# pinellolab/GRAFIMO

Hardware: AMD Instinct MI355X
Metric: scored haplotype k-mers/sec (higher is better)
Workload: dtype int32

## Files before the change

grafimo_amd/_native.py:

```python
import ctypes
import os

import numpy as np

_HERE = os.path.dirname(os.path.abspath(__file__))
LIB_PATH = os.environ.get("GRAFIMO_HIP_LIB") or os.path.join(_HERE, "csrc", "libgrafimo_hip.so")

GFM_OK = 0
GFM_ERR_INVALID = -1
GFM_ERR_ASSERT = -2
GFM_ERR_HIP = -3
GFM_ERR_NOMEM = -4
GFM_ERR_NODEVICE = -5
GFM_ERR_IO = -6
GFM_ERR_OVERFLOW = -7
GFM_NO_SELECT = 2**31 - 1
GFM_FLAG_RESET_HITS = 1
GFM_FLAG_CLEAR_HIST = 2
GFM_FLAG_CALLER_ORDERS_REUSE = 4
GFM_MAX_WIDTH = 64
GFM_BEST_ROW_BITS = 44
GFM_GRAPH_FORWARD_ONLY = 1
GFM_TSV_NO_NODEPATH = 1
GFM_WORKSPACE_RING = 4
# ... 15 lines not shown
P = ctypes.POINTER

PROTOTYPES = {
    "gfm_abi_version": (c_int, []),
    "gfm_last_error": (ctypes.c_char_p, []),
    "gfm_device_count": (c_int, [P(c_int)]),
    "gfm_set_device": (c_int, [c_int]),
    "gfm_compute_log_odds": (c_int, [c_void_p, c_int, c_void_p, c_void_p]),
    "gfm_scale_pwm": (c_int, [c_void_p, c_int, c_void_p, P(c_int), P(c_int), P(c_int), P(c_double)]),
    "gfm_comp_pval_mat": (c_int, [c_void_p, c_int, c_void_p, c_void_p]),
    "gfm_comp_pval_mat_many": (c_int, [c_int, c_void_p, c_void_p, c_void_p, c_void_p]),
    "gfm_motif_create": (c_int, [c_void_p, c_int, c_void_p, c_int, c_int, c_double, c_void_p, P(c_void_p)]),
    "gfm_motif_create_many": (c_int, [c_int, c_void_p, c_void_p, c_void_p, c_void_p, c_void_p, c_void_p, c_void_p,
                                      c_void_p]),
    "gfm_motif_destroy": (None, [c_void_p]),
    "gfm_motif_width": (c_int, [c_void_p]),
    "gfm_motif_table_len": (c_int, [c_void_p]),
    "gfm_motif_score_range": (c_int, [c_void_p, P(c_i32), P(c_i32)]),
    "gfm_motif_tables": (c_int, [c_void_p, c_void_p, c_void_p]),
    "gfm_motif_pvalue_cutoff": (c_int, [c_void_p, c_double, P(c_i32)]),
    "gfm_motif_annotate": (c_int, [c_void_p, c_void_p, c_i64, c_void_p, c_void_p]),
    "gfm_score_kmers": (c_int, [c_void_p, c_void_p, c_i64, c_void_p, c_void_p, c_i32, c_i64,
                                c_void_p, c_i64, c_void_p, ctypes.c_uint32, c_void_p, c_void_p]),
    "gfm_score_kmers_multi": (c_int, [c_void_p, c_int, c_void_p, c_i64, c_void_p, c_void_p, c_void_p, c_i64,
                                      c_void_p, c_void_p, c_void_p, ctypes.c_uint32, c_void_p]),
    "gfm_score_kmers_multi_plan": (c_int, [c_void_p, c_int, c_void_p, c_void_p, c_void_p]),
    "gfm_profile_enable": (c_int, [c_void_p, c_int, c_int]),
    "gfm_profile_read": (c_int, [c_void_p, c_void_p, c_int, P(c_int)]),
    "gfm_profile_mark_tail": (c_int, [c_void_p, c_void_p]),
    "gfm_profile_read_tail": (c_int, [c_void_p, c_void_p, c_int, P(c_int)]),
    "gfm_calibrate_stream": (c_int, [c_int, c_i64, c_int, c_int, P(c_double), P(c_double)]),
    "gfm_qvalue_table": (c_int, [c_void_p, c_void_p, c_double, c_int, c_void_p, c_void_p, c_void_p,
                                 ctypes.c_uint32, c_void_p]),
    "gfm_qvalue_table_multi": (c_int, [c_void_p, c_int, c_void_p, c_double, c_int, c_void_p, c_void_p, c_void_p,
                                       ctypes.c_uint32, c_void_p]),
    "gfm_select_hits": (c_int, [c_void_p, c_void_p, c_i64, c_void_p, c_i64, c_void_p, c_i64, c_void_p,
                                ctypes.c_uint32, c_void_p]),
    "gfm_select_hits_from": (c_int, [c_void_p, c_void_p, c_i64, c_void_p, c_i64, c_void_p, c_i64, c_void_p,
                                     c_void_p, c_i64, c_void_p, c_void_p]),
    "gfm_region_ids": (c_int, [c_void_p, c_i32, c_i64, c_void_p, c_void_p]),
    "gfm_region_best": (c_int, [c_void_p, c_i64, c_void_p, c_i32, c_void_p, c_i32, c_void_p, c_i64, c_void_p, c_void_p]),
    "gfm_locus_max_workspace": (c_i64, [c_i64]),
    "gfm_locus_max": (c_int, [c_void_p, c_i64, c_void_p, c_i32, c_void_p, c_void_p, c_void_p, c_i32, c_void_p, c_void_p,
                              c_i64, c_void_p, c_void_p]),
    "gfm_scan_host": (c_int, [c_void_p, c_void_p, c_i64, c_double, c_int, c_int, c_i64, c_void_p,
                              c_void_p, c_void_p, c_void_p, c_void_p, P(c_i64)]),
# ... 175 lines not shown
```

grafimo_amd/csrc/grafimo_hip.hip:

```cpp

#include <hip/hip_runtime.h>

#include <algorithm>
#include <atomic>
#include <cmath>
#include <cstdarg>
#include <cstdint>
#include <cstdio>
#include <cstdlib>
#include <cstring>
#include <new>
#include <string>
#include <vector>

#include "grafimo_hip.h"

#define GFM_API extern "C" __attribute__((visibility("default")))

#include "gfm_hit_sort.hpp"
#include "gfm_common.hpp"
#include "gfm_score_kernels.hpp"
#include "gfm_quad_launch.hpp"
#include "gfm_stats_kernels.hpp"

struct gfm_motif {
    int W = 0, L = 0, min_val = 0, scale = 1, ndw = 0;
    double offset = 0.0;
    int lo = 0, hi = 0, nb = 0;
    int hlo = 0, hnb = 0;
    int q_waves = kWavesPerWG;
    int part_nb = 0;
    struct Window { int bins, lo; double mass; };
    std::vector<Window> windows;
    int device = 0;
    int n_cu = 256;
    int max_slabs = 0;
    int sel_slabs = 0;
    int reserve_cus = kReserveCUs;
    size_t lds_bytes = 0;
    std::vector<int64_t> sm;
    double bg[4] = {0, 0, 0, 0};
    std::vector<double> h_ptable;
    unsigned char *d_slab = nullptr;
    uint16_t *d_tab = nullptr;
    unsigned *d_ftab = nullptr;
    double *d_pmf = nullptr;
    double *d_ptable = nullptr;
    unsigned *d_partials[kWorkspaces] = {};
    unsigned *d_spill[kWorkspaces] = {};
    long long *d_resid[kWorkspaces] = {};
    int *d_resid_n[kWorkspaces] = {};
    QWork *d_qwork = nullptr;
    double *d_qscratch = nullptr;
    hipStream_t q_stream[kQStreams] = {};
    int q_streams_used = 0;
    unsigned long long q_last_use[kQStreams] = {}, q_calls = 0;
    hipEvent_t ev_selected = nullptr;
    hipStream_t sel_last_stream = nullptr;
    bool sel_valid = false;
    HitCtl *d_ctl = nullptr;
    unsigned call_no = 0;
    hipStream_t last_st = nullptr, last_tail = nullptr;
    unsigned same_pair_run = 0;
    hipEvent_t ev_scored[kWorkspaces] = {};
    hipEvent_t ev_posted[kWorkspaces] = {};
    bool posted_valid[kWorkspaces] = {};
    long long *d_sel_resid = nullptr;
    int *d_sel_resid_n = nullptr;
    HitCtl *d_sel_ctl = nullptr;
    unsigned sel_call_no = 0;
    std::vector<hipEvent_t> ev0, ev1;
    int ev_next = 0, ev_used = 0, ev_every = 1;
    unsigned ev_calls = 0;
    std::vector<hipEvent_t> tev0, tev1;
    int ev_last = -1;
    int tail_pending = -1;
    std::vector<int> tail_order;
};

namespace {

int ensure_device()
{
// ... 470 lines not shown
            for (int c = 0; c < 4; ++c) {
                const unsigned fwd = (unsigned)sm[(size_t)row_of_code[c] * W + j];
                const unsigned rc_ = (unsigned)sm[(size_t)row_of_code[c ^ 2] * W + (W - 1 - j)];
                ftab[(size_t)j * 8 + c] = fwd | (rc_ << 16);
            }
    }
    const size_t o_ftab = carve(ftab.size() * sizeof(unsigned));
    const size_t o_pmf = carve(sizeof(double) * (size_t)m->L);
    const size_t o_ptable = carve(sizeof(double) * (size_t)m->L);
    const size_t o_dp = carve(sizeof(double) * 2 * (size_t)m->L);
    const size_t o_qwork = carve(sizeof(QWork) * kQStreams);
    const size_t o_qscratch = carve(sizeof(double) * (size_t)m->L * kQStreams);
    size_t o_partials[kWorkspaces], o_resid[kWorkspaces], o_resid_n[kWorkspaces], o_spill[kWorkspaces];
    for (int i = 0; i < kWorkspaces; ++i) {
        o_partials[i] = carve(sizeof(unsigned) * (size_t)m->max_slabs * (size_t)(m->part_nb + 1));
        o_resid[i] = carve(sizeof(long long) * (size_t)m->max_slabs * kResidPerWG);
        o_resid_n[i] = carve(sizeof(int) * (size_t)m->max_slabs);
    }
    const size_t o_sel_resid = carve(sizeof(long long) * (size_t)m->sel_slabs * kResidPerWG);
    const size_t o_sel_resid_n = carve(sizeof(int) * (size_t)m->sel_slabs);
    const size_t o_zero = slab_bytes;
    for (int i = 0; i < kWorkspaces; ++i) o_spill[i] = carve(sizeof(unsigned) * (size_t)m->nb * (size_t)kSpillCopies);
    const size_t o_ctl = carve(sizeof(HitCtl));
    const size_t o_sel_ctl = carve(sizeof(HitCtl));
    HIP_TRY(hipMalloc(&m->d_slab, slab_bytes));
    HIP_TRY(hipMemsetAsync(m->d_slab + o_zero, 0, slab_bytes - o_zero, nullptr));
    m->d_tab = reinterpret_cast<uint16_t *>(m->d_slab + o_tab);
    m->d_ftab = reinterpret_cast<unsigned *>(m->d_slab + o_ftab);
    m->d_pmf = reinterpret_cast<double *>(m->d_slab + o_pmf);
    m->d_ptable = reinterpret_cast<double *>(m->d_slab + o_ptable);
    m->d_qwork = reinterpret_cast<QWork *>(m->d_slab + o_qwork);
    m->d_qscratch = reinterpret_cast<double *>(m->d_slab + o_qscratch);
    for (int i = 0; i < kWorkspaces; ++i) {
        m->d_partials[i] = reinterpret_cast<unsigned *>(m->d_slab + o_partials[i]);
        m->d_resid[i] = reinterpret_cast<long long *>(m->d_slab + o_resid[i]);
        m->d_resid_n[i] = reinterpret_cast<int *>(m->d_slab + o_resid_n[i]);
        m->d_spill[i] = reinterpret_cast<unsigned *>(m->d_slab + o_spill[i]);
        HIP_TRY(hipEventCreateWithFlags(&m->ev_scored[i], hipEventDisableTiming | hipEventReleaseToDevice));
        HIP_TRY(hipEventCreateWithFlags(&m->ev_posted[i], hipEventDisableTiming | hipEventReleaseToDevice));
    }
    HIP_TRY(hipEventCreateWithFlags(&m->ev_selected, hipEventDisableTiming));
    m->d_sel_resid = reinterpret_cast<long long *>(m->d_slab + o_sel_resid);
    m->d_sel_resid_n = reinterpret_cast<int *>(m->d_slab + o_sel_resid_n);
    m->d_ctl = reinterpret_cast<HitCtl *>(m->d_slab + o_ctl);
    m->d_sel_ctl = reinterpret_cast<HitCtl *>(m->d_slab + o_sel_ctl);
    *d_rows = reinterpret_cast<double *>(m->d_slab + o_dp);

    HIP_TRY(hipMemcpyAsync(m->d_tab, tab.data(), tab.size() * sizeof(uint16_t), hipMemcpyHostToDevice, nullptr));
    HIP_TRY(hipMemcpyAsync(m->d_ftab, ftab.data(), ftab.size() * sizeof(unsigned), hipMemcpyHostToDevice, nullptr));
    return GFM_OK;
}

int motif_finish(gfm_motif *m)
{
    const int W = m->W;
    long long room16, room8;
    score_rooms(W, &room16, &room8);
    constexpr double kWindowMass16 = 0.9999;
    m->q_waves = kWavesPerWG;
    if (m->nb <= room16) {
        m->hnb = m->nb;
    } else if (room16 >= 256 && best_window(m, (int)room16).mass >= kWindowMass16) {
        m->hnb = (int)room16;
    } else {
        m->q_waves = kWavesPerWG / 2;
        m->hnb = (int)std::min<long long>(m->nb, room8);
    }
// ... 190 lines not shown
    if (!m || !cutoff) return fail(GFM_ERR_INVALID, "NULL argument");
    int a = 0, b = m->L;
    while (a < b) {
        const int mid = (a + b) / 2;
        if (m->h_ptable[mid] < threshold) b = mid; else a = mid + 1;
    }
    *cutoff = a;
    return GFM_OK;
}

GFM_API int gfm_motif_annotate(gfm_motif_t m, const int32_t *scores, int64_t n, double *lo_out,
                               double *p_out)
{
    if (!m || (!scores && n)) return fail(GFM_ERR_INVALID, "NULL argument");
    for (int64_t i = 0; i < n; ++i) {
        const int s = scores[i];
        if (s < 0 || s >= m->L) return fail(GFM_ERR_INVALID, "score %d outside the table", s);
        if (lo_out) lo_out[i] = ((double)s / (double)m->scale) + ((double)m->W * m->offset);
        if (p_out) p_out[i] = m->h_ptable[s];
    }
    return GFM_OK;
}

GFM_API int gfm_score_kmers(gfm_motif_t m, const uint8_t *d_kmers, int64_t n, int32_t *d_scores,
                            uint64_t *d_hist, int32_t select_cutoff, int64_t row_base,
                            int64_t *d_hit_rows, int64_t hit_capacity, uint64_t *d_hit_count,
                            uint32_t flags, void *stream, void *tail_stream)
{
    if (!m) return fail(GFM_ERR_INVALID, "motif is NULL");
    if (n < 0) return fail(GFM_ERR_INVALID, "negative row count");
    hipStream_t st = static_cast<hipStream_t>(stream);
    hipStream_t tail = tail_stream ? static_cast<hipStream_t>(tail_stream) : st;
    const bool split = tail != st;
    if (n == 0) {
        if ((flags & GFM_FLAG_RESET_HITS) && d_hit_count) {
            if (split) {
                HIP_TRY(hipEventRecord(m->ev_scored[0], st));
                HIP_TRY(hipStreamWaitEvent(tail, m->ev_scored[0], 0));
            }
            HIP_TRY(hipMemsetAsync(d_hit_count, 0, sizeof(uint64_t), tail));
        }
        return GFM_OK;
    }
    if (!d_kmers) return fail(GFM_ERR_INVALID, "NULL device buffer");
    {
        int dev = -1;
        HIP_TRY(hipGetDevice(&dev));
        if (dev != m->device)
            return fail(GFM_ERR_INVALID, "the motif lives on device %d, the current device is %d", m->device, dev);
    }
    if ((reinterpret_cast<uintptr_t>(d_kmers) & 15u) != 0)
        return fail(GFM_ERR_INVALID, "d_kmers must be 16-byte aligned");
    if ((reinterpret_cast<uintptr_t>(d_scores) & 3u) != 0)
        return fail(GFM_ERR_INVALID, "d_scores must be 4-byte aligned");
    if (!d_scores && !d_hist && select_cutoff == GFM_NO_SELECT)
        return fail(GFM_ERR_INVALID, "nothing to do: no scores, no histogram, no selection");
    if (n > (int64_t)kQuadRows * 0x7fffff00ll)
        return fail(GFM_ERR_INVALID, "too many rows for one launch (split the batch)");
    const bool select = select_cutoff != GFM_NO_SELECT;
    if (select && (!d_hit_rows || !d_hit_count))
        return fail(GFM_ERR_INVALID, "selection requested without hit buffers");
    const int use_hist = d_hist ? 1 : 0;
    const long long nchunks = (n + kQuadRows - 1) / kQuadRows;
    const long long want = (nchunks + m->q_waves - 1) / m->q_waves;
// ... 22 lines not shown
    const bool caller_orders = (flags & GFM_FLAG_CALLER_ORDERS_REUSE) && same_owner && m->same_pair_run >= (unsigned)kWorkspaces;
    m->same_pair_run = same_owner ? m->same_pair_run + 1 : 1;
    m->last_st = st;
    m->last_tail = tail;
    if (m->posted_valid[ws] && !caller_orders)
        HIP_TRY(hipStreamWaitEvent(st, m->ev_posted[ws], 0));
    if (split && select && !reset && m->posted_valid[ws_prev])
        HIP_TRY(hipStreamWaitEvent(st, m->ev_posted[ws_prev], 0));
    ScoreArgs<1> args{};
    args.store_through = d_scores ? score_store_through(n, 1) : 2;
    fill_motif_args(args.m[0], m, ws, slot, use_hist, m->hlo, m->hnb, select_cutoff, d_scores,
                    reinterpret_cast<long long *>(d_hit_rows), hit_capacity,
                    reset ? nullptr : reinterpret_cast<unsigned long long *>(d_hit_count));
    hipEvent_t scored = split ? m->ev_scored[ws] : nullptr;
    int rc = dispatch_quad(m->W, 1, m, d_kmers, n, row_base, &args, m->lds_bytes, nslabs, m->q_waves, st, false,
                           split ? &scored : nullptr);
    if (rc) return rc;
    if (split) HIP_TRY(hipStreamWaitEvent(tail, scored, 0));
    m->tail_pending = -1;
    if (split && m->ev_last >= 0 && !m->tev0.empty()) {
        HIP_TRY(hipEventRecord(m->tev0[m->ev_last], tail));
        m->tail_pending = m->ev_last;
    }
    rc = launch_post(m, m->d_partials[ws], nslabs, reinterpret_cast<unsigned long long *>(d_hist),
                     m->hlo, m->hnb, m->d_spill[ws], m->d_resid[ws], m->d_resid_n[ws], select ? nslabs : 0, m->d_ctl, slot,
                     reinterpret_cast<long long *>(d_hit_rows), hit_capacity,
                     reinterpret_cast<unsigned long long *>(d_hit_count), tail);
    if (rc) return rc;
    if (split) {
        HIP_TRY(hipEventRecord(m->ev_posted[ws], tail));
        m->posted_valid[ws] = true;
    } else {
        m->posted_valid[ws] = false;
    }
    return GFM_OK;
}

GFM_API int gfm_score_kmers_multi(const gfm_motif_t *motifs, int n_motifs, const uint8_t *d_kmers,
                                  int64_t n, int32_t *const *d_scores, uint64_t *const *d_hist,
                                  const int32_t *select_cutoffs, int64_t row_base,
                                  int64_t *const *d_hit_rows, const int64_t *hit_capacity,
                                  uint64_t *const *d_hit_count, uint32_t flags, void *stream)
{
    if (!motifs || n_motifs < 1) return fail(GFM_ERR_INVALID, "NULL argument");
    if (n < 0) return fail(GFM_ERR_INVALID, "negative row count");
    hipStream_t st = static_cast<hipStream_t>(stream);
    const bool reset = (flags & GFM_FLAG_RESET_HITS) != 0;
    bool no_scores = d_scores == nullptr;
    if (d_scores) {
        int n_null = 0;
        for (int i = 0; i < n_motifs; ++i) n_null += d_scores[i] ? 0 : 1;
        if (n_null != 0 && n_null != n_motifs) return fail(GFM_ERR_INVALID, "d_scores: every entry or none (scores are stored for all motifs of a call or for none)");
        no_scores = n_null == n_motifs;
    }
    for (int i = 0; i < n_motifs; ++i) {
        if (!motifs[i]) return fail(GFM_ERR_INVALID, "motif %d is NULL", i);
        if (motifs[i]->W != motifs[0]->W)
            return fail(GFM_ERR_INVALID, "motifs of one batched launch must share their width (%d vs %d)",
// ... 161 lines not shown
        HIP_TRY(hipEventElapsedTime(&h_ms[i], m->tev0[slot], m->tev1[slot]));
    }
    *n_out = used;
    m->tail_order.clear();
    return GFM_OK;
}

GFM_API int gfm_profile_read(gfm_motif_t m, float *h_ms, int capacity, int *n_out)
{
    if (!m || !n_out || (!h_ms && capacity)) return fail(GFM_ERR_INVALID, "NULL argument");
    const int slots = (int)m->ev0.size();
    const int used = std::min(m->ev_used, capacity);
    for (int i = 0; i < used; ++i) {
        const int slot = ((m->ev_next - m->ev_used + i) % slots + slots) % slots;
        HIP_TRY(hipEventSynchronize(m->ev1[slot]));
        HIP_TRY(hipEventElapsedTime(&h_ms[i], m->ev0[slot], m->ev1[slot]));
    }
    *n_out = used;
    m->ev_used = 0;
    return GFM_OK;
}

namespace {
int launch_qtables(const gfm_motif_t *motifs, int count, uint64_t *const *d_hist, double threshold, int on_qvalue,
                   double *const *d_qtable, int32_t *const *d_cutoff, uint64_t *const *d_nrows, uint32_t flags,
                   hipStream_t st)
{
    QJobs jobs{};
    jobs.threshold = threshold;
    jobs.on_qvalue = on_qvalue;
    int max_blk = 0;
    for (int k = 0; k < count; ++k) {
        gfm_motif *m = motifs[k];
        QJob &q = jobs.j[k];
        q.hist = reinterpret_cast<const unsigned long long *>(d_hist[k]);
        q.ptable = m->d_ptable;
        int qs = 0;
        while (qs < m->q_streams_used && m->q_stream[qs] != st) ++qs;
        if (qs == m->q_streams_used) {
            if (qs < kQStreams) {
                ++m->q_streams_used;
            } else {
                qs = 0;
                for (int c = 1; c < kQStreams; ++c)
                    if (m->q_last_use[c] < m->q_last_use[qs]) qs = c;
            }
            m->q_stream[qs] = st;
        }
        m->q_last_use[qs] = ++m->q_calls;
        q.ws = m->d_qwork + qs;
        q.qtable = (d_qtable && d_qtable[k]) ? d_qtable[k] : m->d_qscratch + (size_t)qs * (size_t)m->L;
        q.cutoff = d_cutoff ? d_cutoff[k] : nullptr;
        q.nrows = d_nrows ? reinterpret_cast<unsigned long long *>(d_nrows[k]) : nullptr;
        q.clear = (flags & GFM_FLAG_CLEAR_HIST) ? reinterpret_cast<unsigned long long *>(d_hist[k]) : nullptr;
        q.L = m->L; q.lo = m->lo; q.hi = m->hi; q.min_val = m->min_val;
        q.nblk = (m->nb + kQThreads - 1) / kQThreads;
        max_blk = std::max(max_blk, q.nblk);
    }
    const dim3 grid((unsigned)max_blk, (unsigned)count);
    hipLaunchKernelGGL(q_count_kernel, grid, dim3(kQThreads), 0, st, jobs);
    hipLaunchKernelGGL(q_raw_kernel, grid, dim3(kQThreads), 0, st, jobs);
    hipLaunchKernelGGL(q_final_kernel, grid, dim3(kQThreads), 0, st, jobs);
    HIP_TRY(hipGetLastError());
    return GFM_OK;
}
}

GFM_API int gfm_qvalue_table(gfm_motif_t m, uint64_t *d_hist, double threshold, int on_qvalue,
                             double *d_qtable, int32_t *d_cutoff, uint64_t *d_nrows, uint32_t flags,
                             void *stream)
{
    if (!m || !d_hist) return fail(GFM_ERR_INVALID, "NULL argument");
// ... 239 lines not shown
```

grafimo_amd/device.py:

```python
import ctypes
from collections import OrderedDict
from typing import List, Optional

import numpy as np

from . import _native as nv

RANGE = nv.RANGE


def _torch():
    import torch
    return torch


_FP_WEIGHTS = {}


def _fingerprint(pmf) -> tuple:
    words = np.ascontiguousarray(pmf, dtype=np.float64).view(np.uint64)
    n = len(words)
    if not n:
        return (0, 0, 0)
    w = _FP_WEIGHTS.get(n)
# ... 200 lines not shown
    def fused_views(self, device):
        v = getattr(self, "_fused_views", None)
        w = self.fused_workspace(device)
        if v is None or v[3] is not w:
            torch, L = _torch(), self.L
            v = self._fused_views = (w[:L], w[L:2 * L].view(torch.float64), w[2 * L:2 * L + 1].view(torch.int32)[:1], w)
        return v[:3]

    def score(self, kmers, scores, hist=None, select_cutoff=None, row_base=0, hit_rows=None,
              hit_count=None, stream=None, reset_hits=False, tail_stream=None):
        n = int(kmers.shape[0])
        assert kmers.is_contiguous() and kmers.dtype == _torch().uint8
        assert n == 0 or kmers.shape[1] == self.width
        cut = nv.GFM_NO_SELECT if select_cutoff is None else int(select_cutoff)
        nv.check(nv.lib().gfm_score_kmers(
            self._h, kmers.data_ptr() if n else None, n, scores.data_ptr() if (n and scores is not None) else None,
            hist.data_ptr() if hist is not None else None, cut, int(row_base),
            hit_rows.data_ptr() if hit_rows is not None else None,
            int(hit_rows.numel()) if hit_rows is not None else 0,
            hit_count.data_ptr() if hit_count is not None else None,
            nv.GFM_FLAG_RESET_HITS if reset_hits else 0, _stream_ptr(stream),
            _stream_ptr(tail_stream) if tail_stream is not None else None))

    def qvalue_table(self, hist, threshold, on_qvalue, qtable=None, cutoff=None, nrows=None,
                     stream=None, clear_hist=False):
        nv.check(nv.lib().gfm_qvalue_table(
            self._h, hist.data_ptr(), float(threshold), int(bool(on_qvalue)),
            qtable.data_ptr() if qtable is not None else None,
            cutoff.data_ptr() if cutoff is not None else None,
            nrows.data_ptr() if nrows is not None else None,
            nv.GFM_FLAG_CLEAR_HIST if clear_hist else 0, _stream_ptr(stream)))

    def select_hits(self, scores, cutoff, hit_rows, hit_count, row_base=0, stream=None,
                    reset_hits=False):
        n = int(scores.numel())
        nv.check(nv.lib().gfm_select_hits(self._h, scores.data_ptr() if n else None, n, cutoff.data_ptr(),
                                          int(row_base), hit_rows.data_ptr(), int(hit_rows.numel()),
                                          hit_count.data_ptr(),
                                          nv.GFM_FLAG_RESET_HITS if reset_hits else 0,
                                          _stream_ptr(stream)))

    def select_hits_from(self, scores, cutoff, cand_rows, cand_count, hit_rows, hit_count, row_base=0, stream=None):
        n = int(scores.numel())
        nv.check(nv.lib().gfm_select_hits_from(self._h, scores.data_ptr() if n else None, n, cutoff.data_ptr(),
                                               int(row_base), cand_rows.data_ptr(), int(cand_rows.numel()),
                                               cand_count.data_ptr(), hit_rows.data_ptr(), int(hit_rows.numel()),
# ... 145 lines not shown
```

grafimo_amd/scan.py:

```python
from typing import Optional

import numpy as np

from . import _native as _nv
from .device import DeviceMotif, _torch

HIT_SCORE_BITS = 20


class ScanSlot:

    def __init__(self, dm: DeviceMotif, n_rows: int, hit_capacity: int, device, scores=None):
        torch = _torch()
        self.n_rows = int(n_rows)
        self.hit_capacity = int(hit_capacity)
        self.scores = scores if scores is not None else torch.empty(self.n_rows, dtype=torch.int32, device=device)
        self.hist = torch.zeros(dm.L, dtype=torch.int64, device=device)
        self.qtable = torch.empty(dm.L, dtype=torch.float64, device=device)
        self.cutoff = torch.zeros(1, dtype=torch.int32, device=device)
        self.nrows = torch.zeros(1, dtype=torch.int64, device=device)
        self.hits = torch.zeros(self.hit_capacity + 1, dtype=torch.int64, device=device)
        self.best = None
        self.cand = None
        self.p_cand_count = self.p_cand_rows = None
# ... 96 lines not shown
        torch = _torch()
        lib = self._lib
        dm = self.dm
        slot = self.slots[self._turn % len(self.slots)]
        self._turn += 1
        main = torch.cuda.current_stream(self.device)
        main_p = main.cuda_stream
        tail = self.side if self.side is not None else main
        tail_p = self._side_p if self.side is not None else main_p
        if slot.used:
            if self.host_paced:
                slot.done.synchronize()
            else:
                main.wait_event(slot.done)
        slot.used = True
        if self._score_ring < len(self.slots) and (on_qvalue or self._regions is not None):
            prev = self.slots[(self._turn - 1 - self._score_ring) % len(self.slots)]
            if prev.used and self._turn > self._score_ring:
                prev.done.synchronize()
        n = int(d_kmers.shape[0])
        kp = d_kmers.data_ptr() if n else None
        h = dm.handle
        use_cand = on_qvalue and self.candidates
        if not on_qvalue:
            key = float(threshold)
            cut = self._cutoffs.get(key)
            if cut is None:
                cut = self._cutoffs[key] = dm.pvalue_cutoff(key)
            _nv.check(lib.gfm_score_kmers(h, kp, n, slot.p_scores, slot.p_hist if want_qvalues else None,
                                          cut, int(row_base), slot.p_hit_rows, slot.hit_capacity,
                                          slot.p_hit_count, _nv.GFM_FLAG_RESET_HITS | self._reuse_flag, main_p, tail_p))
        elif not use_cand:
            _nv.check(lib.gfm_score_kmers(h, kp, n, slot.p_scores, slot.p_hist, _nv.GFM_NO_SELECT, 0,
                                          None, 0, None, self._reuse_flag, main_p, tail_p))
        else:
            key = float(threshold)
            cut = self._cutoffs.get(key)
            if cut is None:
                cut = self._cutoffs[key] = dm.pvalue_cutoff(key)
            slot.candidates()
            _nv.check(lib.gfm_score_kmers(h, kp, n, slot.p_scores, slot.p_hist, cut, int(row_base),
                                          slot.p_cand_rows, slot.hit_capacity, slot.p_cand_count,
                                          _nv.GFM_FLAG_RESET_HITS | self._reuse_flag, main_p, tail_p))
        if want_qvalues:
            if self.collective:
                with torch.cuda.stream(tail):
                    torch.distributed.all_reduce(slot.hist, group=self.group)
            _nv.check(lib.gfm_qvalue_table(h, slot.p_hist, float(threshold), int(bool(on_qvalue)),
                                           slot.p_qtable, slot.p_cutoff, slot.p_nrows,
                                           _nv.GFM_FLAG_CLEAR_HIST, tail_p))
        if on_qvalue and not use_cand:
            _nv.check(lib.gfm_select_hits(h, slot.p_scores, n, slot.p_cutoff, int(row_base),
                                          slot.p_hit_rows, slot.hit_capacity, slot.p_hit_count,
                                          _nv.GFM_FLAG_RESET_HITS, tail_p))
        elif on_qvalue:
            _nv.check(lib.gfm_select_hits_from(h, slot.p_scores, n, slot.p_cutoff, int(row_base),
                                               slot.p_cand_rows, slot.hit_capacity, slot.p_cand_count,
                                               slot.p_hit_rows, slot.hit_capacity, slot.p_hit_count, tail_p))
        if self._regions is not None:
            region, n_regions, freq = self._regions
            with torch.cuda.stream(tail):
                slot.best.zero_()
            _nv.check(lib.gfm_region_best(slot.p_scores, n, region.data_ptr(), n_regions,
                                          freq.data_ptr() if freq is not None else None,
                                          0 if on_qvalue else self._cutoffs[float(threshold)],
                                          slot.p_cutoff if on_qvalue else None, int(row_base), slot.best.data_ptr(), tail_p))
        if gather_hits and self.collective:
# ... 196 lines not shown
```

include/grafimo_hip.h:

```cpp
#ifndef GRAFIMO_HIP_H
#define GRAFIMO_HIP_H

#include <stdint.h>

#ifdef __cplusplus
extern "C" {
#endif

#define GFM_ABI_VERSION 12

#define GFM_OK 0
#define GFM_ERR_INVALID (-1)
#define GFM_ERR_ASSERT (-2)
#define GFM_ERR_HIP (-3)
#define GFM_ERR_NOMEM (-4)
#define GFM_ERR_NODEVICE (-5)
#define GFM_ERR_IO (-6)
#define GFM_ERR_OVERFLOW (-7)

#define GFM_MAX_WIDTH 64
#define GFM_NO_SELECT INT32_MAX
#define GFM_FLAG_RESET_HITS 1u
#define GFM_FLAG_CLEAR_HIST 2u
#define GFM_FLAG_CALLER_ORDERS_REUSE 4u
// ... 17 lines not shown
                           const double *h_bgs, double *h_pmf_out);

typedef struct gfm_motif *gfm_motif_t;

int gfm_motif_create(const int64_t *h_score_matrix, int width, const double *h_bg,
                     int min_val, int scale, double offset, const double *h_pmf,
                     gfm_motif_t *out);
int gfm_motif_create_many(int n_motifs, const int64_t *h_score_matrices, const int *widths,
                          const double *h_bgs, const int *min_vals, const int *scales,
                          const double *offsets, const double *const *h_pmfs, gfm_motif_t *out);
void gfm_motif_destroy(gfm_motif_t m);
int gfm_motif_width(gfm_motif_t m);
int gfm_motif_table_len(gfm_motif_t m);
int gfm_motif_score_range(gfm_motif_t m, int32_t *lo, int32_t *hi);
int gfm_motif_tables(gfm_motif_t m, double *h_pmf_out, double *h_ptable_out);
int gfm_motif_pvalue_cutoff(gfm_motif_t m, double threshold, int32_t *cutoff);
int gfm_motif_annotate(gfm_motif_t m, const int32_t *h_scores, int64_t n,
                       double *h_logodds_out, double *h_pvalue_out);

int gfm_score_kmers(gfm_motif_t m, const uint8_t *d_kmers, int64_t n, int32_t *d_scores,
                    uint64_t *d_hist, int32_t select_cutoff, int64_t row_base,
                    int64_t *d_hit_rows, int64_t hit_capacity, uint64_t *d_hit_count,
                    uint32_t flags, void *stream, void *tail_stream);

int gfm_score_kmers_multi(const gfm_motif_t *motifs, int n_motifs, const uint8_t *d_kmers,
                          int64_t n, int32_t *const *d_scores, uint64_t *const *d_hist,
                          const int32_t *select_cutoffs, int64_t row_base,
                          int64_t *const *d_hit_rows, const int64_t *hit_capacity,
                          uint64_t *const *d_hit_count, uint32_t flags, void *stream);

int gfm_score_kmers_multi_plan(const gfm_motif_t *motifs, int n_motifs, const int32_t *with_hist,
                               int32_t *group_size_out, int32_t *waves_out);

int gfm_profile_enable(gfm_motif_t m, int slots, int every);
int gfm_profile_read(gfm_motif_t m, float *h_ms_out, int capacity, int *n_out);
int gfm_profile_mark_tail(gfm_motif_t m, void *stream);
int gfm_profile_read_tail(gfm_motif_t m, float *h_ms_out, int capacity, int *n_out);

int gfm_calibrate_stream(int loads_per_store, int64_t in_bytes, int store_policy, int launches,
                         double *us_per_launch, double *bytes_per_launch);

int gfm_qvalue_table(gfm_motif_t m, uint64_t *d_hist, double threshold, int on_qvalue,
                     double *d_qtable_out, int32_t *d_cutoff_out, uint64_t *d_nrows_out,
                     uint32_t flags, void *stream);
int gfm_qvalue_table_multi(const gfm_motif_t *motifs, int n_motifs, uint64_t *const *d_hist,
                           double threshold, int on_qvalue, double *const *d_qtable_out,
// ... 209 lines not shown
```

Measured before the change: 229.3 billion.

## Fuse histogram reduction, hit compaction and q-value table into one tail kernel

Adds a fused tail kernel that reduces the per-slab histogram partials, drains spill counters and compacts hit rows. The last block to finish, picked by an atomic ticket, then builds the q-value table and cutoff in the same launch. The scan path calls this new entry point whenever q-values are wanted and the scan is not collective, replacing the separate post and qvalue-table launches. This removes a kernel launch and a dependency hop on the tail stream, at the cost of a grid-wide last-block handoff and a q-phase that runs in a single workgroup.

```diff
diff --git a/grafimo_amd/_native.py b/grafimo_amd/_native.py
--- a/grafimo_amd/_native.py
+++ b/grafimo_amd/_native.py
@@ -61,6 +61,9 @@
     "gfm_motif_annotate": (c_int, [c_void_p, c_void_p, c_i64, c_void_p, c_void_p]),
     "gfm_score_kmers": (c_int, [c_void_p, c_void_p, c_i64, c_void_p, c_void_p, c_i32, c_i64,
                                 c_void_p, c_i64, c_void_p, ctypes.c_uint32, c_void_p, c_void_p]),
+    "gfm_score_kmers_q": (c_int, [c_void_p, c_void_p, c_i64, c_void_p, c_void_p, c_i32, c_i64,
+                                  c_void_p, c_i64, c_void_p, c_double, c_int, c_void_p, c_void_p, c_void_p,
+                                  ctypes.c_uint32, c_void_p, c_void_p]),
     "gfm_score_kmers_multi": (c_int, [c_void_p, c_int, c_void_p, c_i64, c_void_p, c_void_p, c_void_p, c_i64,
                                       c_void_p, c_void_p, c_void_p, ctypes.c_uint32, c_void_p]),
     "gfm_score_kmers_multi_plan": (c_int, [c_void_p, c_int, c_void_p, c_void_p, c_void_p]),
diff --git a/grafimo_amd/csrc/gfm_tail_kernels.hpp b/grafimo_amd/csrc/gfm_tail_kernels.hpp
--- /dev/null
+++ b/grafimo_amd/csrc/gfm_tail_kernels.hpp
@@ -0,0 +1,261 @@
+#pragma once
+
+#include "gfm_score_kernels.hpp"
+#include "gfm_stats_kernels.hpp"
+
+namespace {
+
+#ifndef GFM_TAIL_VARIANT
+#define GFM_TAIL_VARIANT 0
+#endif
+constexpr int kTailBinsPerThread = (GFM_TAIL_VARIANT & 4) ? 4 : 1;
+constexpr int kTailThreads = 256;
+constexpr int kTailWaves = kTailThreads / kWave;
+constexpr int kTailLdsWords = 2 * kTailWaves;
+constexpr int kQBinsPerLane = 8;
+constexpr int kQChunk = kWave * kQBinsPerLane;
+static_assert(kResidPerWG % kTailThreads == 0, "a hit block loads its slab in whole rounds");
+
+struct TailJob {
+    PostJob p;
+    const double *ptable;
+    double *qtable;
+    int *cutoff;
+    unsigned long long *nrows;
+    unsigned long long *clear;
+    unsigned *ticket;
+    double threshold;
+    int on_qvalue, L, qlo, qhi;
+};
+
+__device__ inline double tail_wave_min(double m)
+{
+#pragma unroll
+    for (int d = 32; d > 0; d >>= 1) m = fmin(m, __shfl_xor(m, d));
+    return m;
+}
+
+__device__ inline void
+q_phase(const unsigned long long *hist, const double *__restrict__ ptable, int L, int lo, int hi, int min_val,
+        double threshold, int on_qvalue, double *qtable, int *__restrict__ cutoff_out,
+        unsigned long long *__restrict__ nrows_out, unsigned long long *clear, unsigned long long *sh)
+{
+    const int tid = threadIdx.x, lane = tid & 63, wave = tid >> 6;
+    const int nb = hi - lo + 1;
+    const int per = (nb + kTailWaves * kQChunk - 1) / (kTailWaves * kQChunk) * kQChunk;
+    const int nch = per / kQChunk;
+    const int a = lo + wave * per;
+    const bool n_outside = min_val < lo || min_val > hi;
+    const unsigned long long n_rows_N = n_outside ? hist[min_val] : 0ull;
+    unsigned long long t = 0;
+    for (int c = 0; c < nch; ++c) {
+#pragma unroll
+        for (int i = 0; i < kQBinsPerLane; ++i) {
+            const int j = a + c * kQChunk + i * kWave + lane;
+            const unsigned long long v = hist[min(j, hi)];
+            t += j <= hi ? v : 0ull;
+        }
+    }
+#pragma unroll
+    for (int d = 32; d > 0; d >>= 1) t += __shfl_xor(t, d);
+    if (lane == 0) sh[wave] = t;
+    __syncthreads();
+    unsigned long long n = n_rows_N, carry = 0;
+#pragma unroll
+    for (int w = 0; w < kTailWaves; ++w) {
+        n += sh[w];
+        if (w > wave) carry += sh[w];
+    }
+    const double nd = (double)n;
+    double wmin = INFINITY;
+    for (int c = nch - 1; c >= 0; --c) {
+        const int j0 = a + c * kQChunk + lane * kQBinsPerLane;
+        unsigned long long h[kQBinsPerLane];
+        double p[kQBinsPerLane];
+#pragma unroll
+        for (int i = 0; i < kQBinsPerLane; ++i) {
+            const int j = j0 + i;
+            h[i] = hist[min(j, hi)];
+            p[i] = ptable[min(j, hi)];
+        }
+        unsigned long long loc = 0;
+#pragma unroll
+        for (int i = 0; i < kQBinsPerLane; ++i) {
+            if (j0 + i > hi) h[i] = 0ull;
+            loc += h[i];
+        }
+        unsigned long long inc = loc;
+#pragma unroll
+        for (int d = 1; d < kWave; d <<= 1) {
+            const unsigned long long v = __shfl_down(inc, d);
+            if (lane + d < kWave) inc += v;
+        }
+        unsigned long long c_ge = carry + (inc - loc);
+        carry += __shfl(inc, 0);
+#pragma unroll
+        for (int i = kQBinsPerLane - 1; i >= 0; --i) {
+            c_ge += h[i];
+            const double raw = h[i] ? p[i] / ((double)c_ge / nd) : INFINITY;
+            if (j0 + i <= hi) qtable[j0 + i] = raw;
+            wmin = fmin(wmin, raw);
+        }
+    }
+    wmin = tail_wave_min(wmin);
+    if (lane == 0) sh[kTailWaves + wave] = (unsigned long long)__double_as_longlong(wmin);
+    __syncthreads();
+    double below = INFINITY, all = INFINITY;
+#pragma unroll
+    for (int w = 0; w < kTailWaves; ++w) {
+        const double v = __longlong_as_double((long long)sh[kTailWaves + w]);
+        all = fmin(all, v);
+        if (w < wave) below = fmin(below, v);
+    }
+    const double base = n_rows_N ? ptable[min_val] / (nd / nd) : INFINITY;
+    double run = fmin(below, base);
+    int first = L;
+    for (int c = 0; c < nch; ++c) {
+        const int j0 = a + c * kQChunk + lane * kQBinsPerLane;
+        double r[kQBinsPerLane], p[kQBinsPerLane];
+#pragma unroll
+        for (int i = 0; i < kQBinsPerLane; ++i) {
+            const int j = j0 + i;
+            r[i] = qtable[min(j, hi)];
+            p[i] = ptable[min(j, hi)];
+        }
+#pragma unroll
+        for (int i = 0; i < kQBinsPerLane; ++i) {
+            if (j0 + i > hi) r[i] = INFINITY;
+            if (i) r[i] = fmin(r[i], r[i - 1]);
+        }
+        double inc = r[kQBinsPerLane - 1];
+#pragma unroll
+        for (int d = 1; d < kWave; d <<= 1) {
+            const double v = __shfl_up(inc, d);
+            if (lane >= d) inc = fmin(inc, v);
+        }
+        double lanes_below = __shfl_up(inc, 1);
+        if (lane == 0) lanes_below = INFINITY;
+        const double under = fmin(run, lanes_below);
+        run = fmin(run, __shfl(inc, kWave - 1));
+#pragma unroll
+        for (int i = 0; i < kQBinsPerLane; ++i) {
+            const int j = j0 + i;
+            if (j <= hi) {
+                const double q = fmin(fmin(r[i], under), 1.0);
+                qtable[j] = q;
+                const double val = on_qvalue ? q : p[i];
+                if (val < threshold) first = min(first, j);
+                if (clear) clear[j] = 0ull;
+            }
+        }
+    }
+    const double q_above = fmin(fmin(base, all), 1.0);
+    for (int jj = tid; jj < lo; jj += kTailThreads) qtable[jj] = fmin(base, 1.0);
+    for (int jj = hi + 1 + tid; jj < L; jj += kTailThreads) qtable[jj] = q_above;
+#pragma unroll
+    for (int d = 32; d > 0; d >>= 1) first = min(first, __shfl_xor(first, d));
+    if (lane == 0) sh[wave] = (unsigned long long)first;
+    __syncthreads();
+    if (tid == 0) {
+#pragma unroll
+        for (int w = 1; w < kTailWaves; ++w) first = min(first, (int)sh[w]);
+        if (cutoff_out) *cutoff_out = first;
+        if (nrows_out) *nrows_out = n;
+        if (clear && n_outside) clear[min_val] = 0ull;
+    }
+}
+
+__global__ void __launch_bounds__(kTailThreads) fused_tail_kernel(const TailJob job)
+{
+    __shared__ unsigned long long sh[kTailLdsWords];
+    const PostJob &q = job.p;
+    const int tid = threadIdx.x, lane = tid & 63, wave = tid >> 6;
+    const int bx = (int)blockIdx.x;
+    if (bx == 0 && tid == 0 && q.hit_slabs == 0 && q.ctl) q.ctl->mid[(q.par + kCtlAhead) % kCtlSlots] = 0ull;
+    if (bx < q.hist_blocks) {
+        const int g0 = (bx / q.bin_blocks) * kSlabsPerGroup;
+        const int g1 = min(g0 + kSlabsPerGroup, q.nslabs);
+        const size_t stride = (size_t)(q.nb + 1);
+        unsigned long long s[kTailBinsPerThread];
+#pragma unroll
+        for (int i = 0; i < kTailBinsPerThread; ++i) s[i] = 0;
+#pragma unroll 8
+        for (int g = g0; g < g1; ++g)
+#pragma unroll
+            for (int i = 0; i < kTailBinsPerThread; ++i) {
+                const int b = ((bx % q.bin_blocks) * kTailBinsPerThread + i) * 256 + tid;
+                const unsigned v = __builtin_nontemporal_load(&q.partials[g * stride + min(b, q.nb)]);
+                s[i] += b <= q.nb ? v : 0u;
+            }
+#pragma unroll
+        for (int i = 0; i < kTailBinsPerThread; ++i) {
+            const int b = ((bx % q.bin_blocks) * kTailBinsPerThread + i) * 256 + tid;
+            if (s[i]) atomicAdd(&q.hist64[b == q.nb ? q.min_val : q.lo + b], s[i]);
+        }
+    } else if (bx < q.hist_blocks + q.spill_blocks) {
+        const int b = (bx - q.hist_blocks) * 256 + tid;
+        if (b < q.spill_n) {
+            unsigned long long v = 0;
+#pragma unroll
+            for (int c = 0; c < kSpillCopies; ++c) {
+                const unsigned x = q.spill[(size_t)c * (size_t)q.spill_n + b];
+                if (x) {
+                    v += x;
+                    q.spill[(size_t)c * (size_t)q.spill_n + b] = 0u;
+                }
+            }
+            if (v) atomicAdd(&q.hist64[q.spill_lo + b], v);
+        }
+    } else {
+        const int g = bx - q.hist_blocks - q.spill_blocks;
+        const long long *slab = q.resid + (size_t)g * kResidPerWG;
+        long long e[kResidPerWG / kTailThreads];
+#pragma unroll
+        for (int i = 0; i < kResidPerWG / kTailThreads; ++i) e[i] = __builtin_nontemporal_load(&slab[i * kTailThreads + tid]);
+        const unsigned long long start = q.ctl->snap[q.par] + q.ctl->mid[q.par];
+        const int cnt = q.resid_n[g];
+        unsigned long long both = 0;
+        for (int k = tid; k < q.hit_slabs; k += kTailThreads) {
+            const unsigned long long v = (unsigned long long)q.resid_n[k];
+            both += v + (k < g ? v << 32 : 0ull);
+        }
+#pragma unroll
+        for (int d = 32; d > 0; d >>= 1) both += __shfl_xor(both, d);
+        if (lane == 0) sh[wave] = both;
+        __syncthreads();
+        both = 0;
+#pragma unroll
+        for (int w = 0; w < kTailWaves; ++w) both += sh[w];
+        const unsigned long long base = start + (both >> 32);
+#pragma unroll
+        for (int i = 0; i < kResidPerWG / kTailThreads; ++i) {
+            const int at = i * kTailThreads + tid;
+            if (at < cnt && (long long)(base + at) < q.hit_cap) __builtin_nontemporal_store(e[i], &q.hit_rows[base + at]);
+        }
+        if (g == 0 && tid == 0) {
+            *q.hit_count = start + (both & 0xffffffffull);
+            q.ctl->mid[(q.par + kCtlAhead) % kCtlSlots] = 0ull;
+        }
+        if (GFM_TAIL_VARIANT & 1) return;
+    }
+    asm volatile("s_waitcnt vmcnt(0)" ::: "memory");
+    __syncthreads();
+    if (tid == 0) {
+        if (!(GFM_TAIL_VARIANT & 2)) __builtin_amdgcn_fence(__ATOMIC_RELEASE, "agent");
+        asm volatile("s_waitcnt vmcnt(0)" ::: "memory");
+        const unsigned drawn = __hip_atomic_fetch_add(job.ticket, 1u, __ATOMIC_RELAXED, __HIP_MEMORY_SCOPE_AGENT);
+        const bool last = drawn == (unsigned)((GFM_TAIL_VARIANT & 1) ? q.hist_blocks + q.spill_blocks : (int)gridDim.x) - 1;
+        if (last) {
+            __hip_atomic_store(job.ticket, 0u, __ATOMIC_RELAXED, __HIP_MEMORY_SCOPE_AGENT);
+            __builtin_amdgcn_fence(__ATOMIC_ACQUIRE, "agent");
+            asm volatile("s_waitcnt vmcnt(0)" ::: "memory");
+        }
+        sh[kTailWaves] = last ? 1ull : 0ull;
+    }
+    __syncthreads();
+    if (!sh[kTailWaves]) return;
+    q_phase(q.hist64, job.ptable, job.L, job.qlo, job.qhi, q.min_val, job.threshold, job.on_qvalue, job.qtable,
+            job.cutoff, job.nrows, job.clear, sh);
+}
+
+}
diff --git a/grafimo_amd/csrc/grafimo_hip.hip b/grafimo_amd/csrc/grafimo_hip.hip
--- a/grafimo_amd/csrc/grafimo_hip.hip
+++ b/grafimo_amd/csrc/grafimo_hip.hip
@@ -22,6 +22,7 @@
 #include "gfm_score_kernels.hpp"
 #include "gfm_quad_launch.hpp"
 #include "gfm_stats_kernels.hpp"
+#include "gfm_tail_kernels.hpp"
 
 struct gfm_motif {
     int W = 0, L = 0, min_val = 0, scale = 1, ndw = 0;
@@ -59,6 +60,7 @@
     hipStream_t sel_last_stream = nullptr;
     bool sel_valid = false;
     HitCtl *d_ctl = nullptr;
+    unsigned *d_ticket = nullptr;
     unsigned call_no = 0;
     hipStream_t last_st = nullptr, last_tail = nullptr;
     unsigned same_pair_run = 0;
@@ -575,6 +577,7 @@
     const size_t o_zero = slab_bytes;
     for (int i = 0; i < kWorkspaces; ++i) o_spill[i] = carve(sizeof(unsigned) * (size_t)m->nb * (size_t)kSpillCopies);
     const size_t o_ctl = carve(sizeof(HitCtl));
+    const size_t o_ticket = carve(sizeof(unsigned) * kWorkspaces);
     const size_t o_sel_ctl = carve(sizeof(HitCtl));
     HIP_TRY(hipMalloc(&m->d_slab, slab_bytes));
     HIP_TRY(hipMemsetAsync(m->d_slab + o_zero, 0, slab_bytes - o_zero, nullptr));
@@ -596,6 +599,7 @@
     m->d_sel_resid = reinterpret_cast<long long *>(m->d_slab + o_sel_resid);
     m->d_sel_resid_n = reinterpret_cast<int *>(m->d_slab + o_sel_resid_n);
     m->d_ctl = reinterpret_cast<HitCtl *>(m->d_slab + o_ctl);
+    m->d_ticket = reinterpret_cast<unsigned *>(m->d_slab + o_ticket);
     m->d_sel_ctl = reinterpret_cast<HitCtl *>(m->d_slab + o_sel_ctl);
     *d_rows = reinterpret_cast<double *>(m->d_slab + o_dp);
 
@@ -832,13 +836,52 @@
     return GFM_OK;
 }
 
-GFM_API int gfm_score_kmers(gfm_motif_t m, const uint8_t *d_kmers, int64_t n, int32_t *d_scores,
-                            uint64_t *d_hist, int32_t select_cutoff, int64_t row_base,
-                            int64_t *d_hit_rows, int64_t hit_capacity, uint64_t *d_hit_count,
-                            uint32_t flags, void *stream, void *tail_stream)
+namespace {
+struct QTail {
+    double threshold;
+    int on_qvalue;
+    double *d_qtable;
+    int32_t *d_cutoff;
+    uint64_t *d_nrows;
+};
+
+int q_scratch_set(gfm_motif *m, hipStream_t st);
+int launch_qtables(const gfm_motif_t *motifs, int count, uint64_t *const *d_hist, double threshold, int on_qvalue,
+                   double *const *d_qtable, int32_t *const *d_cutoff, uint64_t *const *d_nrows, uint32_t flags,
+                   hipStream_t st);
+
+int launch_fused_tail(gfm_motif *m, const PostJob &post, int ws, const QTail &qt, uint32_t flags, hipStream_t st)
+{
+    TailJob job{};
+    job.p = post;
+    {
+        const int groups = post.bin_blocks ? post.hist_blocks / post.bin_blocks : 0;
+        job.p.bin_blocks = (post.nb + 1 + 256 * kTailBinsPerThread - 1) / (256 * kTailBinsPerThread);
+        job.p.hist_blocks = job.p.bin_blocks * groups;
+        job.p.total = job.p.hist_blocks + post.spill_blocks + post.hit_slabs;
+    }
+    job.ptable = m->d_ptable;
+    job.qtable = qt.d_qtable ? qt.d_qtable : m->d_qscratch + (size_t)q_scratch_set(m, st) * (size_t)m->L;
+    job.cutoff = qt.d_cutoff;
+    job.nrows = reinterpret_cast<unsigned long long *>(qt.d_nrows);
+    job.clear = (flags & GFM_FLAG_CLEAR_HIST) ? post.hist64 : nullptr;
+    job.ticket = m->d_ticket + ws;
+    job.threshold = qt.threshold;
+    job.on_qvalue = qt.on_qvalue;
+    job.L = m->L; job.qlo = m->lo; job.qhi = m->hi;
+    hipLaunchKernelGGL(fused_tail_kernel, dim3((unsigned)job.p.total), dim3(kTailThreads), 0, st, job);
+    HIP_TRY(hipGetLastError());
+    return GFM_OK;
+}
+
+int score_kmers(gfm_motif_t m, const uint8_t *d_kmers, int64_t n, int32_t *d_scores,
+                uint64_t *d_hist, int32_t select_cutoff, int64_t row_base,
+                int64_t *d_hit_rows, int64_t hit_capacity, uint64_t *d_hit_count,
+                uint32_t flags, void *stream, void *tail_stream, const QTail *qt)
 {
     if (!m) return fail(GFM_ERR_INVALID, "motif is NULL");
     if (n < 0) return fail(GFM_ERR_INVALID, "negative row count");
+    if (qt && !d_hist) return fail(GFM_ERR_INVALID, "a q-table needs the histogram");
     hipStream_t st = static_cast<hipStream_t>(stream);
     hipStream_t tail = tail_stream ? static_cast<hipStream_t>(tail_stream) : st;
     const bool split = tail != st;
@@ -850,6 +893,9 @@
             }
             HIP_TRY(hipMemsetAsync(d_hit_count, 0, sizeof(uint64_t), tail));
         }
+        if (qt)
+            return launch_qtables(&m, 1, &d_hist, qt->threshold, qt->on_qvalue, &qt->d_qtable, &qt->d_cutoff,
+                                  &qt->d_nrows, flags, tail);
         return GFM_OK;
     }
     if (!d_kmers) return fail(GFM_ERR_INVALID, "NULL device buffer");
@@ -918,10 +964,11 @@
         HIP_TRY(hipEventRecord(m->tev0[m->ev_last], tail));
         m->tail_pending = m->ev_last;
     }
-    rc = launch_post(m, m->d_partials[ws], nslabs, reinterpret_cast<unsigned long long *>(d_hist),
-                     m->hlo, m->hnb, m->d_spill[ws], m->d_resid[ws], m->d_resid_n[ws], select ? nslabs : 0, m->d_ctl, slot,
-                     reinterpret_cast<long long *>(d_hit_rows), hit_capacity,
-                     reinterpret_cast<unsigned long long *>(d_hit_count), tail);
+    const PostJob post = post_job(m, m->d_partials[ws], nslabs, reinterpret_cast<unsigned long long *>(d_hist), m->hlo,
+                                  m->hnb, m->d_spill[ws], m->d_resid[ws], m->d_resid_n[ws], select ? nslabs : 0, m->d_ctl,
+                                  slot, reinterpret_cast<long long *>(d_hit_rows), hit_capacity,
+                                  reinterpret_cast<unsigned long long *>(d_hit_count));
+    rc = qt ? launch_fused_tail(m, post, ws, *qt, flags, tail) : launch_posts(&post, 1, tail);
     if (rc) return rc;
     if (split) {
         HIP_TRY(hipEventRecord(m->ev_posted[ws], tail));
@@ -930,6 +977,27 @@
         m->posted_valid[ws] = false;
     }
     return GFM_OK;
+}
+}
+
+GFM_API int gfm_score_kmers(gfm_motif_t m, const uint8_t *d_kmers, int64_t n, int32_t *d_scores,
+                            uint64_t *d_hist, int32_t select_cutoff, int64_t row_base,
+                            int64_t *d_hit_rows, int64_t hit_capacity, uint64_t *d_hit_count,
+                            uint32_t flags, void *stream, void *tail_stream)
+{
+    return score_kmers(m, d_kmers, n, d_scores, d_hist, select_cutoff, row_base, d_hit_rows, hit_capacity, d_hit_count,
+                       flags, stream, tail_stream, nullptr);
+}
+
+GFM_API int gfm_score_kmers_q(gfm_motif_t m, const uint8_t *d_kmers, int64_t n, int32_t *d_scores,
+                              uint64_t *d_hist, int32_t select_cutoff, int64_t row_base,
+                              int64_t *d_hit_rows, int64_t hit_capacity, uint64_t *d_hit_count,
+                              double threshold, int on_qvalue, double *d_qtable, int32_t *d_cutoff,
+                              uint64_t *d_nrows, uint32_t flags, void *stream, void *tail_stream)
+{
+    const QTail qt{threshold, on_qvalue, d_qtable, d_cutoff, d_nrows};
+    return score_kmers(m, d_kmers, n, d_scores, d_hist, select_cutoff, row_base, d_hit_rows, hit_capacity, d_hit_count,
+                       flags, stream, tail_stream, &qt);
 }
 
 GFM_API int gfm_score_kmers_multi(const gfm_motif_t *motifs, int n_motifs, const uint8_t *d_kmers,
@@ -1137,6 +1205,24 @@
 }
 
 namespace {
+int q_scratch_set(gfm_motif *m, hipStream_t st)
+{
+    int qs = 0;
+    while (qs < m->q_streams_used && m->q_stream[qs] != st) ++qs;
+    if (qs == m->q_streams_used) {
+        if (qs < kQStreams) {
+            ++m->q_streams_used;
+        } else {
+            qs = 0;
+            for (int c = 1; c < kQStreams; ++c)
+                if (m->q_last_use[c] < m->q_last_use[qs]) qs = c;
+        }
+        m->q_stream[qs] = st;
+    }
+    m->q_last_use[qs] = ++m->q_calls;
+    return qs;
+}
+
 int launch_qtables(const gfm_motif_t *motifs, int count, uint64_t *const *d_hist, double threshold, int on_qvalue,
                    double *const *d_qtable, int32_t *const *d_cutoff, uint64_t *const *d_nrows, uint32_t flags,
                    hipStream_t st)
@@ -1150,19 +1236,7 @@
         QJob &q = jobs.j[k];
         q.hist = reinterpret_cast<const unsigned long long *>(d_hist[k]);
         q.ptable = m->d_ptable;
-        int qs = 0;
-        while (qs < m->q_streams_used && m->q_stream[qs] != st) ++qs;
-        if (qs == m->q_streams_used) {
-            if (qs < kQStreams) {
-                ++m->q_streams_used;
-            } else {
-                qs = 0;
-                for (int c = 1; c < kQStreams; ++c)
-                    if (m->q_last_use[c] < m->q_last_use[qs]) qs = c;
-            }
-            m->q_stream[qs] = st;
-        }
-        m->q_last_use[qs] = ++m->q_calls;
+        const int qs = q_scratch_set(m, st);
         q.ws = m->d_qwork + qs;
         q.qtable = (d_qtable && d_qtable[k]) ? d_qtable[k] : m->d_qscratch + (size_t)qs * (size_t)m->L;
         q.cutoff = d_cutoff ? d_cutoff[k] : nullptr;
diff --git a/grafimo_amd/device.py b/grafimo_amd/device.py
--- a/grafimo_amd/device.py
+++ b/grafimo_amd/device.py
@@ -246,6 +246,26 @@
             nv.GFM_FLAG_RESET_HITS if reset_hits else 0, _stream_ptr(stream),
             _stream_ptr(tail_stream) if tail_stream is not None else None))
 
+    def score_q(self, kmers, scores, hist, threshold, on_qvalue, qtable=None, cutoff=None, nrows=None,
+                select_cutoff=None, row_base=0, hit_rows=None, hit_count=None, stream=None, reset_hits=False,
+                tail_stream=None, clear_hist=False):
+        n = int(kmers.shape[0])
+        assert kmers.is_contiguous() and kmers.dtype == _torch().uint8
+        assert n == 0 or kmers.shape[1] == self.width
+        cut = nv.GFM_NO_SELECT if select_cutoff is None else int(select_cutoff)
+        flags = (nv.GFM_FLAG_RESET_HITS if reset_hits else 0) | (nv.GFM_FLAG_CLEAR_HIST if clear_hist else 0)
+        nv.check(nv.lib().gfm_score_kmers_q(
+            self._h, kmers.data_ptr() if n else None, n, scores.data_ptr() if (n and scores is not None) else None,
+            hist.data_ptr(), cut, int(row_base),
+            hit_rows.data_ptr() if hit_rows is not None else None,
+            int(hit_rows.numel()) if hit_rows is not None else 0,
+            hit_count.data_ptr() if hit_count is not None else None,
+            float(threshold), int(bool(on_qvalue)),
+            qtable.data_ptr() if qtable is not None else None,
+            cutoff.data_ptr() if cutoff is not None else None,
+            nrows.data_ptr() if nrows is not None else None,
+            flags, _stream_ptr(stream), _stream_ptr(tail_stream) if tail_stream is not None else None))
+
     def qvalue_table(self, hist, threshold, on_qvalue, qtable=None, cutoff=None, nrows=None,
                      stream=None, clear_hist=False):
         nv.check(nv.lib().gfm_qvalue_table(
diff --git a/grafimo_amd/scan.py b/grafimo_amd/scan.py
--- a/grafimo_amd/scan.py
+++ b/grafimo_amd/scan.py
@@ -142,27 +142,34 @@
         kp = d_kmers.data_ptr() if n else None
         h = dm.handle
         use_cand = on_qvalue and self.candidates
+        fused = want_qvalues and not self.collective
+        if fused:
+            def score(scores, hist, cut, row_base, hit_rows, cap, hit_count, flags):
+                _nv.check(lib.gfm_score_kmers_q(h, kp, n, scores, hist, cut, row_base, hit_rows, cap, hit_count,
+                                                float(threshold), int(bool(on_qvalue)), slot.p_qtable, slot.p_cutoff,
+                                                slot.p_nrows, flags | _nv.GFM_FLAG_CLEAR_HIST, main_p, tail_p))
+        else:
+            def score(scores, hist, cut, row_base, hit_rows, cap, hit_count, flags):
+                _nv.check(lib.gfm_score_kmers(h, kp, n, scores, hist, cut, row_base, hit_rows, cap, hit_count, flags,
+                                              main_p, tail_p))
         if not on_qvalue:
             key = float(threshold)
             cut = self._cutoffs.get(key)
             if cut is None:
                 cut = self._cutoffs[key] = dm.pvalue_cutoff(key)
-            _nv.check(lib.gfm_score_kmers(h, kp, n, slot.p_scores, slot.p_hist if want_qvalues else None,
-                                          cut, int(row_base), slot.p_hit_rows, slot.hit_capacity,
-                                          slot.p_hit_count, _nv.GFM_FLAG_RESET_HITS | self._reuse_flag, main_p, tail_p))
+            score(slot.p_scores, slot.p_hist if want_qvalues else None, cut, int(row_base), slot.p_hit_rows,
+                  slot.hit_capacity, slot.p_hit_count, _nv.GFM_FLAG_RESET_HITS | self._reuse_flag)
         elif not use_cand:
-            _nv.check(lib.gfm_score_kmers(h, kp, n, slot.p_scores, slot.p_hist, _nv.GFM_NO_SELECT, 0,
-                                          None, 0, None, self._reuse_flag, main_p, tail_p))
+            score(slot.p_scores, slot.p_hist, _nv.GFM_NO_SELECT, 0, None, 0, None, self._reuse_flag)
         else:
             key = float(threshold)
             cut = self._cutoffs.get(key)
             if cut is None:
                 cut = self._cutoffs[key] = dm.pvalue_cutoff(key)
             slot.candidates()
-            _nv.check(lib.gfm_score_kmers(h, kp, n, slot.p_scores, slot.p_hist, cut, int(row_base),
-                                          slot.p_cand_rows, slot.hit_capacity, slot.p_cand_count,
-                                          _nv.GFM_FLAG_RESET_HITS | self._reuse_flag, main_p, tail_p))
-        if want_qvalues:
+            score(slot.p_scores, slot.p_hist, cut, int(row_base), slot.p_cand_rows, slot.hit_capacity,
+                  slot.p_cand_count, _nv.GFM_FLAG_RESET_HITS | self._reuse_flag)
+        if want_qvalues and not fused:
             if self.collective:
                 with torch.cuda.stream(tail):
                     torch.distributed.all_reduce(slot.hist, group=self.group)
diff --git a/include/grafimo_hip.h b/include/grafimo_hip.h
--- a/include/grafimo_hip.h
+++ b/include/grafimo_hip.h
@@ -63,6 +63,12 @@
                     uint64_t *d_hist, int32_t select_cutoff, int64_t row_base,
                     int64_t *d_hit_rows, int64_t hit_capacity, uint64_t *d_hit_count,
                     uint32_t flags, void *stream, void *tail_stream);
+
+int gfm_score_kmers_q(gfm_motif_t m, const uint8_t *d_kmers, int64_t n, int32_t *d_scores,
+                      uint64_t *d_hist, int32_t select_cutoff, int64_t row_base,
+                      int64_t *d_hit_rows, int64_t hit_capacity, uint64_t *d_hit_count,
+                      double threshold, int on_qvalue, double *d_qtable_out, int32_t *d_cutoff_out,
+                      uint64_t *d_nrows_out, uint32_t flags, void *stream, void *tail_stream);
 
 int gfm_score_kmers_multi(const gfm_motif_t *motifs, int n_motifs, const uint8_t *d_kmers,
                           int64_t n, int32_t *const *d_scores, uint64_t *const *d_hist,
```

Measured after the change: 168.0 billion. 0.733x the previous value.
